# duburcqa/jiminy

Hardware: AMD Instinct MI355X
Metric: env-steps/s (whole node) ANYmal 18-DoF batch 65536; achieved HBM GB/s vs peak (higher is better)
Workload: dtype f64

## Files before the change

### jiminy_amd/csrc/jm_quad.h

```cpp
#pragma once
#include "jm_kernels.h"

namespace jm
{
template<class Tp> struct QLayout
{
    static constexpr int J_PLC = 0, J_RBI = 12, J_AXIS = 22, J_AXP = 25, J_ROTOR = 28, J_QLO = 29, J_QHI = 30, J_MOTOR = 31, J_ENC = 40;
    static constexpr int QJ = 41;
    static constexpr int C_IDX = 12, C_CS = 13, C_FREL = 14;
    static constexpr int QC = Tp::QHAS_FORCE ? 26 : 14;
    static constexpr int CONTACT = Tp::QN * QJ;
    static constexpr int RAW = CONTACT + Tp::QCL * QC;
    static constexpr int QSTRIDE = (RAW % 2 == 0) ? RAW + 1 : RAW;
    static constexpr int TABLE = 4 * QSTRIDE;
    static constexpr int OFFSET = Layout<Tp>::TOTAL;
    static constexpr int TOTAL = OFFSET + TABLE;
};

JM_DEV int sel4(int k, int c0, int c1, int c2, int c3) { return k == 0 ? c0 : (k == 1 ? c1 : (k == 2 ? c2 : c3)); }

template<class Tp> struct QInfo
{
    static constexpr int N = Tp::QN, NT = Tp::QT;
    static constexpr int NQB = 7 + (NT - 1), NVB = 6 + (NT - 1);
// ... 44 lines not shown
    if (ax == 1) return {c * R.m00 - s * R.m02, R.m01, c * R.m02 + s * R.m00, c * R.m10 - s * R.m12, R.m11, c * R.m12 + s * R.m10,
                         c * R.m20 - s * R.m22, R.m21, c * R.m22 + s * R.m20};
    return {c * R.m00 + s * R.m01, c * R.m01 - s * R.m00, R.m02, c * R.m10 + s * R.m11, c * R.m11 - s * R.m10, R.m12,
            c * R.m20 + s * R.m21, c * R.m21 - s * R.m20, R.m22};
}
template<class T> struct LimbTable
{
    const T * base;
    JM_DEV T operator()(int off) const { return base[off]; }
    JM_DEV V3<T> v3(int o) const { return {base[o], base[o + 1], base[o + 2]}; }
    JM_DEV M3<T> m3(int o) const { return {base[o], base[o + 1], base[o + 2], base[o + 3], base[o + 4], base[o + 5], base[o + 6], base[o + 7], base[o + 8]}; }
    JM_DEV SE3<T> se3(int o) const { return {m3(o), v3(o + 9)}; }
    JM_DEV RBI<T> rbi(int o) const { return {base[o], v3(o + 1), S3<T>{base[o + 4], base[o + 5], base[o + 6], base[o + 7], base[o + 8], base[o + 9]}}; }
};
template<class T, class Tp, int s> JM_DEV V3<T> limb_axis_root(const LimbTable<T> & LT, const M3<T> & Rs_)
{
    constexpr int ax = limb_axis_uniform<Tp>(s);
    if constexpr (ax >= 0)
    {
        if constexpr (limb_axis_negative<Tp>(s)) return LT(s * QLayout<Tp>::QJ + QLayout<Tp>::J_AXIS + ax) * mcol(Rs_, ax);
        else return mcol(Rs_, ax);
    }
    else return Rs_ * LT.v3(s * QLayout<Tp>::QJ + QLayout<Tp>::J_AXIS);
}

template<class T, class X> JM_DEV Sp<T> quad_sum6(Sp<T> a)
{
    return {{X::quad_sum(a.l.x), X::quad_sum(a.l.y), X::quad_sum(a.l.z)}, {X::quad_sum(a.a.x), X::quad_sum(a.a.y), X::quad_sum(a.a.z)}};
}
template<class T, class X> JM_DEV AI<T> quad_sum_ai(const AI<T> & Y)
{
    AI<T> r;
    r.A = {X::quad_sum(Y.A.xx), X::quad_sum(Y.A.xy), X::quad_sum(Y.A.xz), X::quad_sum(Y.A.yy), X::quad_sum(Y.A.yz), X::quad_sum(Y.A.zz)};
    r.B = {X::quad_sum(Y.B.m00), X::quad_sum(Y.B.m01), X::quad_sum(Y.B.m02), X::quad_sum(Y.B.m10), X::quad_sum(Y.B.m11), X::quad_sum(Y.B.m12),
           X::quad_sum(Y.B.m20), X::quad_sum(Y.B.m21), X::quad_sum(Y.B.m22)};
    r.D = {X::quad_sum(Y.D.xx), X::quad_sum(Y.D.xy), X::quad_sum(Y.D.xz), X::quad_sum(Y.D.yy), X::quad_sum(Y.D.yz), X::quad_sum(Y.D.zz)};
    return r;
}
template<class T> JM_DEV Sp<T> operator*(T s, Sp<T> a) { return {s * a.l, s * a.a}; }
template<class T> JM_DEV T dot6(Sp<T> a, Sp<T> b) { return dot(a.l, b.l) + dot(a.a, b.a); }
template<class T> JM_DEV Sp<T> mask6(bool on, Sp<T> a)
{
    const T z = T(0);
    return {{on ? a.l.x : z, on ? a.l.y : z, on ? a.l.z : z}, {on ? a.a.x : z, on ? a.a.y : z, on ? a.a.z : z}};
}
template<class T> JM_DEV AI<T> mask_ai(bool on, const AI<T> & Y)
{
    const T z = T(0);
    AI<T> r;
    r.A = {on ? Y.A.xx : z, on ? Y.A.xy : z, on ? Y.A.xz : z, on ? Y.A.yy : z, on ? Y.A.yz : z, on ? Y.A.zz : z};
    r.B = {on ? Y.B.m00 : z, on ? Y.B.m01 : z, on ? Y.B.m02 : z, on ? Y.B.m10 : z, on ? Y.B.m11 : z, on ? Y.B.m12 : z,
           on ? Y.B.m20 : z, on ? Y.B.m21 : z, on ? Y.B.m22 : z};
    r.D = {on ? Y.D.xx : z, on ? Y.D.xy : z, on ? Y.D.xz : z, on ? Y.D.yy : z, on ? Y.D.yz : z, on ? Y.D.zz : z};
    return r;
}
template<class T> JM_DEV RBI<T> rbi_placed(const M3<T> & R, V3<T> p, const RBI<T> & Y)
{
    return {Y.m, R * Y.c + p, rot_sym(R, Y.I)};
}

template<class T, int SL, int SB> struct StageBuf
{
    T * sl;
    T * sb;
    bool wb;
    JM_DEV T getl(int row) const { return sl[row * SL]; }
    JM_DEV void putl(int row, T x) const { sl[row * SL] = x; }
    JM_DEV T getb(int row) const { return sb[row * SB]; }
    JM_DEV void putb(int row, T x) const { if (wb) sb[row * SB] = x; }
};
template<class Tp> struct QRows
{
    static constexpr int N = Tp::QN, NQB = QInfo<Tp>::NQB, NVB = QInfo<Tp>::NVB;
    static constexpr int Q0B = 0, V0B = NQB, ACCVB = V0B + NVB, ACCAB = ACCVB + NVB, KVB = ACCAB + NVB;
    static constexpr int Q0L = 0, V0L = N, ACCVL = 2 * N, ACCAL = 3 * N, KVL = 4 * N;
#ifdef JM_QUAD_LEAN
    static constexpr bool LONG = true;
#else
    static constexpr bool LONG = N > 4;
#endif
    static constexpr bool CMD_LDS = true;
    static constexpr int CMDL = 5 * N, NL = CMD_LDS ? 6 * N : 5 * N;
    static constexpr int CMDB = KVB + NVB, NB = CMD_LDS ? CMDB + Tp::QT : CMDB;
};

template<class Tp> struct QSplitRows
{
    using R = QRows<Tp>;
    static constexpr int N = Tp::QN, NQB = QInfo<Tp>::NQB, NVB = QInfo<Tp>::NVB;
    static constexpr int CURQL = R::NL, CURVL = CURQL + N, DDQL = CURVL + N, STATUSL = DDQL + N, CXL = STATUSL + 1, NCX = 16;
    static constexpr int NL = CXL + NCX;
    static constexpr int CURQB = R::NB, CURVB = CURQB + NQB, DDQB = CURVB + NVB, NB = DDQB + NVB;
    static constexpr int TILE = NL * 64 + NB * 16;
};

template<class T> JM_DEV void add6(T * base, unsigned B, unsigned r, unsigned row0, Sp<T> f)
{
    const unsigned o = row0 * B + r;
    base[o] += f.l.x; base[o + B] += f.l.y; base[o + 2 * B] += f.l.z;
    base[o + 3 * B] += f.a.x; base[o + 4 * B] += f.a.y; base[o + 5 * B] += f.a.z;
}
template<class T> JM_DEV void put6(T * base, unsigned B, unsigned r, unsigned row0, Sp<T> f)
{
    const unsigned o = row0 * B + r;
    base[o] = f.l.x; base[o + B] = f.l.y; base[o + 2 * B] = f.l.z;
    base[o + 3 * B] = f.a.x; base[o + 4 * B] = f.a.y; base[o + 5 * B] = f.a.z;
}

template<class T, int FL, class MP> JM_DEV void motor_law(MP && mp, T cmd, T vjnt, T & um, T & ut)
{
    const T red = mp(0), elim = mp(1), vlim = mp(2), islope = mp(3);
    const T vmot = red * vjnt;
    um = cmd;
    if constexpr ((FL & JM_MOTOR_EFFORT_LIMIT) != 0)
    {
        T emin = -elim, emax = elim;
        if constexpr ((FL & JM_MOTOR_VELOCITY_LIMIT) != 0)
        {
            const T vdelta = elim * islope;
            const bool on = vdelta > T(0);
            const T vthr = fmax_(vlim - vdelta, T(0));
            const T inv = rcp_(on ? vlim - vthr : T(1));
            emin *= on ? clamp_((vlim + vmot) * inv, T(0), T(1)) : T(1);
            emax *= on ? clamp_((vlim - vmot) * inv, T(0), T(1)) : T(1);
        }
        um = clamp_(um, emin, emax);
    }
    ut = red * um;
    if constexpr ((FL & JM_MOTOR_FRICTION) != 0)
    {
        const T fds = mp(8);
        if (vjnt > T(0)) ut += mp(4) * vjnt + mp(6) * tanh_(fds * vjnt);
        else ut += mp(5) * vjnt + mp(7) * tanh_(fds * vjnt);
    }
}

template<class Tp> struct QIdx
{
    int rq[Tp::QN], rv[Tp::QN], rm[Tp::QN];
    bool has[Tp::QN];
    int nc;
    int attach;
};
template<class Tp> JM_DEV QIdx<Tp> quad_indices(int k)
{
    QIdx<Tp> ix;
    static_for<0, Tp::QN>([&](auto sc) {
        constexpr int s = decltype(sc)::value;
        constexpr auto J = [](int kk) { return Tp::limb_joint[kk][s] < 0 ? 1 : Tp::limb_joint[kk][s]; };
        ix.rq[s] = sel4(k, Tp::idx_q[J(0)], Tp::idx_q[J(1)], Tp::idx_q[J(2)], Tp::idx_q[J(3)]);
        ix.rv[s] = sel4(k, Tp::idx_v[J(0)], Tp::idx_v[J(1)], Tp::idx_v[J(2)], Tp::idx_v[J(3)]);
        ix.rm[s] = sel4(k, Tp::limb_motor[0][s] < 0 ? 0 : Tp::limb_motor[0][s], Tp::limb_motor[1][s] < 0 ? 0 : Tp::limb_motor[1][s],
                        Tp::limb_motor[2][s] < 0 ? 0 : Tp::limb_motor[2][s], Tp::limb_motor[3][s] < 0 ? 0 : Tp::limb_motor[3][s]);
        ix.has[s] = sel4(k, s < Tp::limb_len[0], s < Tp::limb_len[1], s < Tp::limb_len[2], s < Tp::limb_len[3]) != 0;
    });
    ix.nc = sel4(k, Tp::limb_ncontact[0], Tp::limb_ncontact[1], Tp::limb_ncontact[2], Tp::limb_ncontact[3]);
    ix.attach = sel4(k, Tp::limb_attach[0], Tp::limb_attach[1], Tp::limb_attach[2], Tp::limb_attach[3]);
    return ix;
}

struct NoModelLane
{
    template<class V> JM_DEV V rbi(int, const V & c) const { return c; }
    template<class V> JM_DEV V plc_p(int, const V & c) const { return c; }
};
template<class T> struct ModelLane
// ... 303 lines not shown
    constexpr int ax = limb_axis_uniform<Tp>(s);
    if constexpr (ax >= 0)
    {
        R = mul_rot_axis(R * plc.R, ax, c, sn);
        if constexpr (limb_axis_negative<Tp>(s)) a = LT(o + Q::J_AXIS + ax) * mcol(R, ax);
        else a = mcol(R, ax);
    }
    else
    {
        a = R * LT.v3(o + Q::J_AXP);
        R = R * (plc.R * rot_rodrigues(LT.v3(o + Q::J_AXIS), c, sn));
    }
}
template<class T, class Tp, int s, class MA = NoModelLane>
JM_DEV void limb_unwind(const LimbTable<T> & LT, T c, T sn, M3<T> & R, V3<T> & p, const MA & ma = MA{}, int k = 0)
{
    using Q = QLayout<Tp>;
    constexpr int o = s * Q::QJ;
    SE3<T> plc = LT.se3(o + Q::J_PLC);
    if constexpr (!std::is_same<MA, NoModelLane>::value)
        plc.p = ma.plc_p(sel4(k, Tp::limb_joint[0][s], Tp::limb_joint[1][s], Tp::limb_joint[2][s], Tp::limb_joint[3][s]), plc.p);
    constexpr int ax = limb_axis_uniform<Tp>(s);
    M3<T> Rq;
    if constexpr (ax >= 0) Rq = mul_rot_axis(R, ax, c, -sn);
    else Rq = R * rot_rodrigues(LT.v3(o + Q::J_AXIS), c, -sn);
    R = mul_bt(Rq, plc.R);
    p = p - R * plc.p;
}

template<class T> JM_DEV Sp<T> applied_wrench_on(const BatchArgs<T> & A, int jq, const M3<T> & R1, const M3<T> & Rj, V3<T> pj,
                                                 unsigned B32, unsigned r32, T te)
{
    Sp<T> f = zero6<T>();
    for (int i = 0; i < A.applied_k; ++i)
    {
        if (A.applied_joint[i] != jq) continue;
        V3<T> F = zero3<T>(), M = zero3<T>();
        if (A.applied)
        {
            const unsigned o = (unsigned)(6 * i) * B32 + r32;
            F = {A.applied[o], A.applied[o + B32], A.applied[o + 2 * B32]};
            M = {A.applied[o + 3 * B32], A.applied[o + 4 * B32], A.applied[o + 5 * B32]};
        }
        if (A.proc_off > 0) add_process_forces(A, i, te, (long long)B32, (long long)r32, F, M);
        const V3<T> p = pj + Rj * V3<T>{A.applied_p[3 * i], A.applied_p[3 * i + 1], A.applied_p[3 * i + 2]};
        const V3<T> fl = tmul(R1, F);
        f.l = f.l + fl;
        f.a = f.a + tmul(R1, M) + cross(p, fl);
    }
    return f;
}
template<class T> JM_DEV Sp<T> applied_root_wrench(const BatchArgs<T> & A, const M3<T> & R1, unsigned B32, unsigned r32, T te)
{
    return applied_wrench_on(A, 1, R1, ident3<T>(), zero3<T>(), B32, r32, te);
}
template<class T> JM_DEV Sp<T> wrench_to_joint(const M3<T> & Rj, V3<T> pj, Sp<T> w)
{
    return {tmul(Rj, w.l), tmul(Rj, w.a - cross(pj, w.l))};
}

template<class T, class Tp> struct QExtra
{
    T tau_l[Tp::QN], tau_b[Tp::QT], uemit_l[Tp::QN], uemit_b[Tp::QT];
    bool motors_on;
    const int32_t * flags;
    const T * lam;
    int nb;
};
struct NoKeep { static constexpr bool ON = false; };
template<class T, class Tp> struct TrunkStore;
template<class T, class Tp> struct QKeep
{
    static constexpr bool ON = true;
    V3<T> ps[Tp::QN], as[Tp::QN];
    Sp<T> Us[Tp::QN];
    T dinv[Tp::QN];
    M3<T> Rt;
    Sp<T> vtip, atip;
    M3<T> R1; V3<T> p1;
    Sp<T> agf1;
    T rootL[6][6], rootdinv[6];
};

template<class T, class Tp, class X, bool EMIT, class SB, int CFM = 0, class KEEP = NoKeep, bool GEN = false, bool DYN = true>
JM_DEV void quad_eval(CPtr<T> P, const LimbTable<T> & LT, const BatchArgs<T> & A, unsigned r, int k, const QIdx<Tp> & ix,
                      const SB & S_, const T * qb, const T * vb_, const T * ql, const T * vl_, const T * cmdb_, const T * cmdl_,
                      bool sensors, T * ddqb, T * ddq, int & status, const QExtra<T, Tp> * ex = nullptr, KEEP * keep = nullptr,
                      TrunkStore<T, Tp> * ts_out = nullptr, T te = T(0))
{
    (void)te;
    using RW = QRows<Tp>;
    auto vlq = [&](int s) -> T { if constexpr (RW::LONG) return S_.getl(RW::KVL + s); else return vl_[s]; };
    auto vbq = [&](int i) -> T { if constexpr (RW::LONG) return S_.getb(RW::KVB + i); else return vb_[i]; };
    auto cmdlq = [&](int s) -> T { if constexpr (RW::CMD_LDS) return S_.getl(RW::CMDL + s); else return cmdl_[s]; };
    auto cmdbq = [&](int t) -> T { if constexpr (RW::CMD_LDS) return S_.getb(RW::CMDB + t); else return cmdb_[t]; };
    constexpr bool emit = EMIT;
    using L = Layout<Tp>;
    using Q = QLayout<Tp>;
    using I = QInfo<Tp>;
    constexpr int N = Tp::QN, NT = Tp::QT;
    constexpr int FL = Tp::motor_flags[0];
    const unsigned B32 = (unsigned)A.B;
    unsigned r32 = r;
    JM_OPAQUE(r32);
    unsigned Bg = B32, rg = r32;
    if constexpr (GEN)
        if (A.lane_map) { rg = (unsigned)A.lane_map[r32]; Bg = (unsigned)A.B_full; }
    const bool lead = (k == 0);
    const bool emit_sens = emit && sensors;
    const bool want_energy = emit && A.energy;
    if constexpr (Tp::QHAS_ENC)
        if (emit_sens && A.encoder)
        {
            static_for<0, N>([&](auto sc) {
                constexpr int s = decltype(sc)::value;
                const int si = sel4(k, Tp::limb_enc[0][s], Tp::limb_enc[1][s], Tp::limb_enc[2][s], Tp::limb_enc[3][s]);
                T pos = ql[s], vel = vlq(s);
                if constexpr (Tp::QENC_SIDE == 0)
                {
                    const T red = LT(s * Q::QJ + Q::J_ENC);
                    pos *= red;
                    vel *= red;
                }
                if (ix.has[s])
                {
                    A.encoder[(unsigned)(2 * si) * B32 + r32] = pos;
                    A.encoder[(unsigned)(2 * si + 1) * B32 + r32] = vel;
                }
            });
            if (lead)
                static_for<1, NT>([&](auto tc) {
                    constexpr int t = decltype(tc)::value;
                    constexpr int si = Tp::trunk_enc[t];
                    T pos = qb[6 + t], vel = vbq(5 + t);
                    if constexpr (Tp::QENC_SIDE == 0) { pos *= P[L::ENC + si]; vel *= P[L::ENC + si]; }
                    A.encoder[(unsigned)(2 * si) * B32 + r32] = pos;
                    A.encoder[(unsigned)(2 * si + 1) * B32 + r32] = vel;
                });
        }
    const M3<T> R1 = quat_to_matrix(qb[3], qb[4], qb[5], qb[6]);
    const V3<T> p1 = {qb[0], qb[1], qb[2]};
    V3<T> p1g = p1;
    if constexpr (GEN)
        if (A.ground_off) { p1g.x += A.ground_off[rg]; p1g.y += A.ground_off[Bg + rg]; }
    const V3<T> g = ld_v3<T>(P, L::OPT), gw = ld_v3<T>(P, L::OPT + 3);
    const Sp<T> v1 = {{vb_[0], vb_[1], vb_[2]}, {vb_[3], vb_[4], vb_[5]}};
    const Sp<T> agf1 = actinv_motion(SE3<T>{R1, p1}, Sp<T>{-g, -gw});
    TrunkStore<T, Tp> TS;
#ifdef JM_HOST_EMU
    std::memset(&TS, 0xFF, sizeof(TS));
#endif
    SE3<T> Xatt;
    Sp<T> vatt;
    using MA = std::conditional_t<GEN, ModelLane<T>, NoModelLane>;
    MA ma;
    if constexpr (GEN) ma = ModelLane<T>{A.model_lane, Bg, rg};
    auto limb_joint_of = [&](auto sc) {
        constexpr int s = decltype(sc)::value;
        return sel4(k, Tp::limb_joint[0][s], Tp::limb_joint[1][s], Tp::limb_joint[2][s], Tp::limb_joint[3][s]);
    };
    (void)limb_joint_of;
    trunk_fk_store<T, Tp, X, MA>(P, k, ix, qb, vb_, TS, Xatt, vatt, status, ma);
#ifdef JM_OUTPUT_KEEP_KIN
    constexpr bool UNWIND = QRows<Tp>::LONG;
#else
    constexpr bool UNWIND = QRows<Tp>::LONG || !DYN;
#endif
    constexpr bool REWIND = UNWIND;
    M3<T> Rs[UNWIND ? 1 : N];
    V3<T> ps[N];
    T cq[UNWIND ? N : 1], sq[UNWIND ? N : 1];
    M3<T> Rtip;
    V3<T> ptip;
    Sp<T> vtip;
    if constexpr (UNWIND) limb_fk_tip<T, Tp, MA>(LT, Xatt, vatt, ql, vl_, cq, sq, Rtip, ptip, vtip, status, ma, k);
    else
    {
        limb_fk<T, Tp, MA>(LT, ix, Xatt, vatt, ql, vl_, Rs, ps, vtip, status, ma, k);
        Rtip = Rs[N - 1]; ptip = ps[N - 1];
    }
    if constexpr (CFM != 0) status &= ~JM_LANE_OUT_OF_BOUNDS;
    Sp<T> fext = zero6<T>();
    {
        const M3<T> Rt = Rtip;
        const V3<T> pt = ptip;
        const Sp<T> vt = vtip;
        Sp<T> fext_loc = zero6<T>(), fsens = zero6<T>();
        T fmax2 = T(0);
        auto one_contact = [&](int c) {
            const int oc = Q::CONTACT + c * Q::QC;
            const SE3<T> fr = LT.se3(oc);
            const V3<T> pc = Rt * fr.p + pt;
            T depth = p1.z + dot(V3<T>{R1.m20, R1.m21, R1.m22}, pc);
            V3<T> nG = {T(0), T(0), T(1)};
            if constexpr (GEN && CFM == 0)
                if (A.ground_h)
                {
                    const V3<T> pW = R1 * pc + p1g;
                    T hG;
                    ground_profile(A, pW.x, pW.y, hG, nG);
                    depth = (pW.z - hG) * nG.z;
                }
            const bool active = c < ix.nc;
            Sp<T> fl = zero6<T>();
            if constexpr (CFM == 0)
            {
                if (active && depth < T(0))
                {
                    const V3<T> vW = R1 * (vt.l + cross(vt.a, pc));
                    V3<T> fW;
                    if constexpr (GEN) fW = contact_law_n<T, Tp>(P, nG, depth, vW, A.friction ? A.friction[rg] : T(-1));
                    else fW = contact_law<T, Tp>(P, depth, vW);
                    const V3<T> fR = tmul(R1, fW);
                    fext.l = fext.l + fR;
                    fext.a = fext.a + cross(pc, fR);
                    fmax2 = fmax_(fmax2, dot(fW, fW));
                    if (emit)
                    {
                        fl.l = tmul(Rt, fR);
                        fl.a = cross(fr.p, fl.l);
                    }
                }
            }
            else if constexpr (CFM == 2)
            {
                (void)depth;
                if (active)
                {
                    const unsigned ci = (unsigned)(int)LT(oc + Q::C_IDX);
                    if (ex->flags[((unsigned)ex->nb + ci) * B32 + r32] & 1)
                    {
                        const unsigned o = ((unsigned)ex->nb + 4u * ci) * B32 + r32;
                        T dep_;
                        const M3<T> Mc = contact_frame<GEN>(A, R1, p1g, pc, dep_);
                        const V3<T> fR = tmul(Mc, V3<T>{ex->lam[o], ex->lam[o + B32], ex->lam[o + 2 * B32]});
                        const V3<T> tR = ex->lam[o + 3 * B32] * V3<T>{Mc.m20, Mc.m21, Mc.m22};
                        fext.l = fext.l + fR;
                        fext.a = fext.a + cross(pc, fR) + tR;
                        if (emit)
                        {
                            fl.l = tmul(Rt, fR);
                            fl.a = cross(fr.p, fl.l) + tmul(Rt, tR);
                        }
                    }
                }
            }
            else { (void)depth; }
            if (emit && active)
            {
                fext_loc = fext_loc + fl;
                const Sp<T> cf = actinv_force(fr, fl);
                if (A.contact_forces) put6(A.contact_forces, B32, r32, 6 * (unsigned)(int)LT(oc + Q::C_IDX), cf);
                if constexpr (Tp::QHAS_CS)
                    if (sensors && A.contact)
                    {
                        const unsigned o = 3 * (unsigned)(int)LT(oc + Q::C_CS) * B32 + r32;
                        A.contact[o] = cf.l.x; A.contact[o + B32] = cf.l.y; A.contact[o + 2 * B32] = cf.l.z;
                    }
                if constexpr (Tp::QHAS_FORCE)
                    if (sensors && A.force) fsens = fsens + act_force(LT.se3(oc + Q::C_FREL), cf);
            }
        };
        if constexpr (Tp::QCL <= 2)
            static_for<0, Tp::QCL>([&](auto cc) { one_contact(decltype(cc)::value); });
        else
        {
#pragma nounroll
            for (int c = 0; c < Tp::QCL; ++c) one_contact(c);
        }
        if constexpr (EMIT && CFM == 0)
            if ((A.mode == MODE_START || A.mode == MODE_RESET) && fmax2 > T(1e10)) status |= JM_LANE_FORCE_OVERFLOW;
        if (emit)
        {
            if (A.f_external)
            {
                if (lead)
                {
                    put6(A.f_external, B32, r32, 0, zero6<T>());
                    static_for<0, NT>([&](auto tc) { put6(A.f_external, B32, r32, 6 * Tp::trunk_joint[decltype(tc)::value], zero6<T>()); });
                    if constexpr (GEN)
                        if (A.applied_k > 0) put6(A.f_external, B32, r32, 6 * Tp::trunk_joint[0], applied_root_wrench(A, R1, Bg, rg, te));
                }
                static_for<0, N>([&](auto sc) {
                    constexpr int s = decltype(sc)::value;
                    const int j = sel4(k, Tp::limb_joint[0][s], Tp::limb_joint[1][s], Tp::limb_joint[2][s], Tp::limb_joint[3][s]);
                    const bool tip = sel4(k, s == Tp::limb_len[0] - 1, s == Tp::limb_len[1] - 1, s == Tp::limb_len[2] - 1, s == Tp::limb_len[3] - 1) != 0;
                    if (ix.has[s]) put6(A.f_external, B32, r32, 6 * (unsigned)j, mask6(tip, fext_loc));
                });
            }
            if constexpr (Tp::QHAS_FORCE)
                if (sensors && A.force)
                {
                    const int si = sel4(k, Tp::limb_force[0], Tp::limb_force[1], Tp::limb_force[2], Tp::limb_force[3]);
                    if (si >= 0) put6(A.force, B32, r32, 6 * (unsigned)si, fsens);
                }
        }
    }
    constexpr bool MOTORS_IN_SWEEP = QRows<Tp>::LONG && !EMIT && DYN;
    T u[N], ut[NT];
    auto limb_motor = [&](auto sc) -> T {
        constexpr int s = decltype(sc)::value;
        constexpr int o = s * Q::QJ + Q::J_MOTOR;
        T um, ue;
        motor_law<T, FL>([&](int i) { return LT(o + i); }, cmdlq(s), vlq(s), um, ue);
        T ueff = ue, ue_out = ue;
        if constexpr (CFM != 0)
        {
            ueff = (ex->motors_on ? ue : T(0)) + ex->tau_l[s];
            ue_out = ue + ex->uemit_l[s];
        }
        if (emit && ix.has[s])
        {
            if (A.u_motor) A.u_motor[(unsigned)ix.rm[s] * B32 + r32] = um;
            if (A.u) A.u[(unsigned)ix.rv[s] * B32 + r32] = ue_out;
            if constexpr (Tp::QHAS_EFF)
                if (sensors && A.effort)
                {
                    const int si = sel4(k, Tp::limb_eff[0][s], Tp::limb_eff[1][s], Tp::limb_eff[2][s], Tp::limb_eff[3][s]);
                    A.effort[(unsigned)si * B32 + r32] = um;
                }
        }
        return ueff;
    };
    auto trunk_motor = [&](auto tc) -> T {
        constexpr int t = decltype(tc)::value;
        constexpr int m = Tp::trunk_motor[t];
        constexpr int o = L::MOTOR + JM_MOTOR_NPARAMS * m;
        T um, ue;
        motor_law<T, FL>([&](int i) { return P[o + i]; }, cmdbq(t), vbq(5 + t), um, ue);
        T ueff = ue, ue_out = ue;
        if constexpr (CFM != 0)
        {
            ueff = (ex->motors_on ? ue : T(0)) + ex->tau_b[t];
            ue_out = ue + ex->uemit_b[t];
        }
        if (emit && lead)
        {
            if (A.u_motor) A.u_motor[(unsigned)m * B32 + r32] = um;
            if (A.u) A.u[(unsigned)Tp::idx_v[Tp::trunk_joint[t]] * B32 + r32] = ue_out;
            if constexpr (Tp::QHAS_EFF)
                if (sensors && A.effort) A.effort[(unsigned)Tp::trunk_eff[t] * B32 + r32] = um;
        }
        return ueff;
    };
    if constexpr (!MOTORS_IN_SWEEP)
    {
        static_for<0, N>([&](auto sc) { u[decltype(sc)::value] = limb_motor(sc); });
        ut[0] = T(0);
        static_for<1, NT>([&](auto tc) { ut[decltype(tc)::value] = trunk_motor(tc); });
    }
    if (emit && A.u && lead)
    {
#pragma unroll
        for (int i = 0; i < 6; ++i) A.u[(unsigned)(Tp::idx_v[1] + i) * B32 + r32] = T(0);
    }
    JM_REFRESH();
    constexpr bool KEEP_SC = !QRows<Tp>::LONG;
    V3<T> as[N];
    Sp<T> Ss[KEEP_SC ? N : 1], cs[KEEP_SC ? N : 1];
    Sp<T> Us[N];
    T dinv[N];
    AI<T> Ia;
    Sp<T> pa = zero6<T>();
    T kin = T(0), rot = T(0), msum = T(0);
    V3<T> mc = zero3<T>();
    {
        Sp<T> vcur = vtip;
        M3<T> Rcur = Rtip;
        V3<T> pcur = ptip;
        static_rfor<0, N>([&](auto sc) {
            constexpr int s = decltype(sc)::value;
            constexpr int o = s * Q::QJ;
            if constexpr (!UNWIND) { Rcur = Rs[s]; pcur = ps[s]; }
            else if constexpr (!REWIND) ps[s] = pcur;
            if constexpr (!DYN) return;
            const RBI<T> Y = rbi_placed(Rcur, pcur, ma.rbi(GEN ? limb_joint_of(sc) : 0, LT.rbi(o + Q::J_RBI)));
            const V3<T> a = limb_axis_root<T, Tp, s>(LT, Rcur);
            const Sp<T> S = {cross(pcur, a), a};
            Sp<T> f = cross_mf(vcur, rbi_mul(Y, vcur));
            if constexpr (s == N - 1) { f = f - fext; Ia = ai_from_rbi(Y); }
            else { f = f + pa; Ia = ai_from_rbi(Y) + Ia; }
            if constexpr (GEN)
                if (A.applied_k > 0)
                {
                    const Sp<T> w = applied_wrench_on(A, limb_joint_of(sc), R1, Rcur, pcur, Bg, rg, te);
                    f = f - w;
                    if constexpr (EMIT)
                        if (A.f_external && ix.has[s]) add6(A.f_external, B32, r32, 6u * (unsigned)limb_joint_of(sc), wrench_to_joint(Rcur, pcur, w));
                }
            if (want_energy)
            {
                kin += rbi_vtiv(Y, vcur);
                mc = mc + Y.m * Y.c;
                msum += Y.m;
                rot += LT(o + Q::J_ROTOR) * vlq(s) * vlq(s);
            }
            const Sp<T> vj = vlq(s) * S;
            vcur = vcur - vj;
            const Sp<T> c = cross_mm(vcur, vj);
            if constexpr (MOTORS_IN_SWEEP) u[s] = limb_motor(sc);
            const T uj = u[s] - dot6(S, f);
            const Sp<T> U = ai_mul(Ia, S);
            const T D = dot6(S, U) + LT(o + Q::J_ROTOR);
            const T di = rcp_(D);
            ai_rank1_sub(Ia, U, di);
            const Sp<T> Ya = ai_mul(Ia, c);
            const T ud = uj * di;
            pa = {f.l + Ya.l + ud * U.l, f.a + Ya.a + ud * U.a};
            Us[s] = U; dinv[s] = di; u[s] = uj;
            if constexpr (KEEP_SC) { Ss[s] = S; cs[s] = c; }
            else if constexpr (!REWIND) as[s] = a;
            if constexpr (KEEP::ON) { keep->ps[s] = pcur; keep->as[s] = a; keep->Us[s] = U; keep->dinv[s] = di; }
            if constexpr (UNWIND && s > 0) limb_unwind<T, Tp, s, MA>(LT, cq[s], sq[s], Rcur, pcur, ma, k);
        });
    }
    AI<T> accA[NT];
    Sp<T> accF[NT];
#ifdef JM_HOST_EMU
    std::memset(accA, 0xFF, sizeof(accA)); std::memset(accF, 0xFF, sizeof(accF));
#endif
    if constexpr (DYN)
    static_for<0, NT>([&](auto tc) {
        constexpr int t = decltype(tc)::value;
        if constexpr (I::limb_at(t))
        {
            if constexpr (I::uniform_attach) { accA[t] = quad_sum_ai<T, X>(Ia); accF[t] = quad_sum6<T, X>(pa); }
            else
            {
                const bool mine = ix.attach == t;
                accA[t] = quad_sum_ai<T, X>(mask_ai(mine, Ia));
                accF[t] = quad_sum6<T, X>(mask6(mine, pa));
            }
        }
// ... 762 lines not shown
                static_for<0, NQB>([&](auto ic) { S.putb(R::Q0B + decltype(ic)::value, qb[decltype(ic)::value]); });
                static_for<0, NVB>([&](auto ic) {
                    constexpr int i = decltype(ic)::value;
                    S.putb(R::V0B + i, vb[i]); S.putb(R::KVB + i, vb[i]); S.putb(R::ACCVB + i, T(0)); S.putb(R::ACCAB + i, T(0));
                });
                static_for<0, N>([&](auto sc) {
                    constexpr int s = decltype(sc)::value;
                    S.putl(R::Q0L + s, ql[s]); S.putl(R::V0L + s, vl[s]); S.putl(R::KVL + s, vl[s]);
                    S.putl(R::ACCVL + s, T(0)); S.putl(R::ACCAL + s, T(0));
                });
                if (last)
                {
                    if (lead)
                    {
                        static_for<0, NQB>([&](auto ic) { A.q[(unsigned)I::qrow(decltype(ic)::value) * B32 + rr] = qb[decltype(ic)::value]; });
                        static_for<0, NVB>([&](auto ic) { A.v[(unsigned)I::vrow(decltype(ic)::value) * B32 + rr] = vb[decltype(ic)::value]; });
                    }
                    static_for<0, N>([&](auto sc) {
                        constexpr int s = decltype(sc)::value;
                        if (ix.has[s])
                        {
                            A.q[(unsigned)ix.rq[s] * B32 + rr] = ql[s];
                            A.v[(unsigned)ix.rv[s] * B32 + rr] = vl[s];
                        }
                    });
                }
            }
        }
    };
    unsigned rr = r32;
    if constexpr (QCON)
    {
        const int start_passes = INIT == 1 ? 4 : (INIT == 0 ? (A.mode == MODE_REFRESH ? -1 : 0) :
                                 ((A.mode == MODE_START || A.mode == MODE_RESET) ? 4 : (A.mode == MODE_REFRESH ? -1 : 0)));
        if constexpr (PH != 0)
        {
            const int e = split_e;
            const int st = (e < pre) ? -1 : (rk4 ? ((e - pre) & 3) : 3);
            const bool last = e == n_evals - 1;
            if constexpr (PH == 1)
            {
                advance(st, last, rr);
                static_for<0, NQB>([&](auto ic) { S.putb(SR::CURQB + decltype(ic)::value, qb[decltype(ic)::value]); });
                static_for<0, NVB>([&](auto ic) { S.putb(SR::CURVB + decltype(ic)::value, vb[decltype(ic)::value]); });
                static_for<0, N>([&](auto sc) {
                    S.putl(SR::CURQL + decltype(sc)::value, ql[decltype(sc)::value]);
                    S.putl(SR::CURVL + decltype(sc)::value, vl[decltype(sc)::value]);
                });
            }
            quad_eval_con<T, Tp, X, StageBuf<T, SL, SB>, CAPC, GEN, PH, INIT>(P, LT, A, *C, *V, rr, k, ix, S, qb, vb, ql, vl, cmdb, cmdl, last,
                                    !stepping || A.update_sensors != 0, ddqb, ddq, status,
                                    INIT == 1 ? 4 : (INIT == 0 ? 0 : ((A.mode == MODE_START || A.mode == MODE_RESET) ? 4 : 0)));
            if (PH == 1 || !last)
            {
                S.putl(SR::STATUSL, (T)status);
                if constexpr (PH == 2)
                {
                    static_for<0, NVB>([&](auto ic) { S.putb(SR::DDQB + decltype(ic)::value, ddqb[decltype(ic)::value]); });
                    static_for<0, N>([&](auto sc) { S.putl(SR::DDQL + decltype(sc)::value, ddq[decltype(sc)::value]); });
                }
                return;
            }
        }
        else
        {
#pragma nounroll
        for (int e = 0; e < n_evals; ++e)
        {
            const int st = (e < pre) ? -1 : (rk4 ? ((e - pre) & 3) : 3);
            const bool last = e == n_evals - 1;
            JM_REFRESH();
            rr = r32;
            JM_OPAQUE(rr);
            advance(st, last, rr);
            if (stepping) stage_time(st);
            quad_eval_con<T, Tp, X, StageBuf<T, SL, SB>, CAPC, GEN, 0, INIT>(P, LT, A, *C, *V, rr, k, ix, S, qb, vb, ql, vl, cmdb, cmdl, last && A.mode != MODE_DYNAMICS,
                                    (!stepping && A.mode != MODE_REFRESH) || A.update_sensors != 0, ddqb, ddq, status,
                                    start_passes, te);
        }
        }
    }
    else
    {
    if (stepping)
    {
#pragma nounroll
        for (int e = 0; e < n_evals; ++e)
        {
            const int st = (e < pre) ? -1 : (rk4 ? ((e - pre) & 3) : 3);
            JM_REFRESH();
            rr = r32;
            JM_OPAQUE(rr);
            CPtr<T> Pl = P;
            if constexpr (R::LONG && !GEN) JM_OPAQUE_S(Pl);
            advance(st, e == n_evals - 1, rr);
            stage_time(st);
            quad_eval<T, Tp, X, false, StageBuf<T, SL, SB>, 0, NoKeep, GEN>(Pl, LT, A, rr, k, ix, S, qb, vb, ql, vl, cmdb, cmdl, false, ddqb, ddq, status,
                                                                             nullptr, nullptr, nullptr, te);
        }
    }
    else
    {
        JM_REFRESH();
        rr = r32;
        JM_OPAQUE(rr);
        advance(-1, true, rr);
        quad_eval<T, Tp, X, false, StageBuf<T, SL, SB>, 0, NoKeep, GEN>(P, LT, A, rr, k, ix, S, qb, vb, ql, vl, cmdb, cmdl, false, ddqb, ddq, status,
                                                                         nullptr, nullptr, nullptr, te);
    }
    if (A.mode != MODE_DYNAMICS)
    {
        JM_REFRESH();
        rr = r32;
        JM_OPAQUE(rr);
        static_for<0, NQB>([&](auto ic) { qb[decltype(ic)::value] = S.getb(R::Q0B + decltype(ic)::value); });
        static_for<0, NVB>([&](auto ic) { vb[decltype(ic)::value] = S.getb(R::V0B + decltype(ic)::value); });
        static_for<0, N>([&](auto sc) { ql[decltype(sc)::value] = S.getl(R::Q0L + decltype(sc)::value); vl[decltype(sc)::value] = S.getl(R::V0L + decltype(sc)::value); });
        quad_eval<T, Tp, X, true, StageBuf<T, SL, SB>, 0, NoKeep, GEN, false>(P, LT, A, rr, k, ix, S, qb, vb, ql, vl, cmdb, cmdl,
                                  (!stepping && A.mode != MODE_REFRESH) || A.update_sensors != 0, ddqb, ddq, status,
                                  nullptr, nullptr, nullptr, te);
    }
    }
    {
        T * adst = (A.mode == MODE_DYNAMICS) ? A.a_out : A.a;
        if (lead) static_for<0, NVB>([&](auto ic) { adst[(unsigned)I::vrow(decltype(ic)::value) * B32 + rr] = ddqb[decltype(ic)::value]; });
        static_for<0, N>([&](auto sc) { if (ix.has[decltype(sc)::value]) adst[(unsigned)ix.rv[decltype(sc)::value] * B32 + rr] = ddq[decltype(sc)::value]; });
        if (A.mode != MODE_DYNAMICS)
        {
            const int stq = X::quad_or(status);
            if (A.status && lead) A.status[rr] = (A.mode == MODE_REFRESH) ? (A.status[rr] | stq) : stq;
            if constexpr (GEN && PH == 0)
                if (stepping && lead && A.proc_off > 0) proc_block(A).lane_time()[rr] = tl;
            if constexpr (QCON)
            if (A.joint_forces || A.centroidal)
            {
                JM_REFRESH();
                static_for<0, NQB>([&](auto ic) { qb[decltype(ic)::value] = S.getb(R::Q0B + decltype(ic)::value); });
                static_for<0, NVB>([&](auto ic) { vb[decltype(ic)::value] = S.getb(R::V0B + decltype(ic)::value); });
                static_for<0, N>([&](auto sc) { ql[decltype(sc)::value] = S.getl(R::Q0L + decltype(sc)::value); vl[decltype(sc)::value] = S.getl(R::V0L + decltype(sc)::value); });
                QExtra<T, Tp> ex;
                ex.flags = C->flags;
                ex.nb = qcon_first_contact_row<Tp>();
                ex.lam = C->data + (size_t)qcon_first_lambda_row<Tp>() * B32;
                quad_extra_terms<T, Tp, X, 2, GEN>(P, LT, A, rr, k, ix, qb, vb, ql, vl, ddqb, ddq, &ex, te);
            }
        }
    }
}

#ifndef JM_HOST_EMU
struct DppQuad
{
    template<int CTRL> static __device__ __forceinline__ int mov(int v) { return __builtin_amdgcn_update_dpp(0, v, CTRL, 0xf, 0xf, true); }
    template<int CTRL> static __device__ __forceinline__ double perm(double x)
    {
        const int lo = mov<CTRL>(__double2loint(x)), hi = mov<CTRL>(__double2hiint(x));
        return __hiloint2double(hi, lo);
    }
    template<int CTRL> static __device__ __forceinline__ float perm(float x) { return __int_as_float(mov<CTRL>(__float_as_int(x))); }
    template<int CTRL> static __device__ __forceinline__ int perm(int x) { return mov<CTRL>(x); }
    template<class T> static __device__ __forceinline__ T quad_sum(T x)
    {
        x = x + perm<0xB1>(x);
        x = x + perm<0x4E>(x);
        return x;
    }
    template<int LANE, class T> static __device__ __forceinline__ T bcast(T x) { return perm<LANE * 0x55>(x); }
    static __device__ __forceinline__ int quad_or(int x)
    {
        x |= mov<0xB1>(x);
        x |= mov<0x4E>(x);
        return x;
    }
    template<int CTRL, class T> static __device__ __forceinline__ T perm_(T x) { return perm<CTRL>(x); }
    static __device__ __forceinline__ bool wave_any(bool p) { return __builtin_amdgcn_ballot_w64(p) != 0ull; }
    static __device__ __forceinline__ double max_abs(double a, double b)
    {
        double r;
        asm("v_max_f64 %0, %1, |%2|" : "=v"(r) : "v"(a), "v"(b));
        return r;
    }
    static __device__ __forceinline__ double max_(double a, double b)
    {
        double r;
        asm("v_max_f64 %0, %1, %2" : "=v"(r) : "v"(a), "v"(b));
        return r;
    }
    static __device__ __forceinline__ float max_abs(float a, float b) { return fmaxf(a, fabsf(b)); }
    static __device__ __forceinline__ float max_(float a, float b) { return fmaxf(a, b); }
#ifdef JM_SYNC_FENCE
    static __device__ __forceinline__ void sync() { __builtin_amdgcn_fence(__ATOMIC_ACQ_REL, "wavefront"); }
#else
    static __device__ __forceinline__ void sync() {}
#endif
    static __device__ __forceinline__ void fence() { __builtin_amdgcn_fence(__ATOMIC_SEQ_CST, "workgroup"); }
    static __device__ __forceinline__ void table_ready() { __syncthreads(); }
};

template<class T, class Tp> constexpr int quad_block_waves()
{
#ifdef JM_QUAD_BLOCK_WAVES
    return JM_QUAD_BLOCK_WAVES;
#endif
    constexpr long per_wave = (long)sizeof(T) * (QRows<Tp>::NL * 64 + QRows<Tp>::NB * 16);
    constexpr long table = (long)sizeof(T) * QLayout<Tp>::TABLE;
    int best = 1, best_resident = 0;
    for (int w = 1; w <= 4; w *= 2)
    {
        long blocks = (160L * 1024) / (table + w * per_wave);
// ... 52 lines not shown
```

Measured before the change: 455.1 million.

## Emit quad sensor, contact and motor outputs during final dynamics eval

For short-limb, single-trunk quadruped configurations, the last RK stage (or the single eval) now writes encoder, contact-force, f_external, force-sensor, u and u_motor outputs directly. It also stashes the summed tip wrench in LDS. The later emit pass (QE_OUT) then reuses that wrench and skips the contact and motor recomputation. Accelerations are written before the output pass. The aim is to remove redundant contact and actuator work in the refresh/emit evaluation. The cost is extra branches, register pressure and code size inside the hot eval loop.

```diff
diff --git a/jiminy_amd/csrc/jm_quad.h b/jiminy_amd/csrc/jm_quad.h
--- a/jiminy_amd/csrc/jm_quad.h
+++ b/jiminy_amd/csrc/jm_quad.h
@@ -150,6 +150,7 @@
     static constexpr bool CMD_LDS = true;
     static constexpr int CMDL = 5 * N, NL = CMD_LDS ? 6 * N : 5 * N;
     static constexpr int CMDB = KVB + NVB, NB = CMD_LDS ? CMDB + Tp::QT : CMDB;
+    static constexpr int FEXTL = ACCVL;
 };
 
 template<class Tp> struct QSplitRows
@@ -619,13 +620,25 @@
     T rootL[6][6], rootdinv[6];
 };
 
-template<class T, class Tp, class X, bool EMIT, class SB, int CFM = 0, class KEEP = NoKeep, bool GEN = false, bool DYN = true>
+enum { QE_OFF = 0, QE_LOOP = 1, QE_SINGLE = 2, QE_OUT = 3 };
+template<class Tp, bool GEN, bool QCON, int CFM = 0, class KEEP = NoKeep> constexpr bool quad_early_outputs()
+{
+#ifdef JM_QUAD_NO_EARLY_OUTPUTS
+    return false;
+#endif
+    return !GEN && !QCON && CFM == 0 && !KEEP::ON && !QRows<Tp>::LONG && Tp::QT == 1 && 2 * Tp::QN >= 6;
+}
+
+template<class T, class Tp, class X, bool EMIT, class SB, int CFM = 0, class KEEP = NoKeep, bool GEN = false, bool DYN = true, int EARLY = QE_OFF>
 JM_DEV void quad_eval(CPtr<T> P, const LimbTable<T> & LT, const BatchArgs<T> & A, unsigned r, int k, const QIdx<Tp> & ix,
                       const SB & S_, const T * qb, const T * vb_, const T * ql, const T * vl_, const T * cmdb_, const T * cmdl_,
                       bool sensors, T * ddqb, T * ddq, int & status, const QExtra<T, Tp> * ex = nullptr, KEEP * keep = nullptr,
-                      TrunkStore<T, Tp> * ts_out = nullptr, T te = T(0))
+                      TrunkStore<T, Tp> * ts_out = nullptr, T te = T(0), bool early = false)
 {
     (void)te;
+    (void)early;
+    constexpr bool EARLY_DYN = EARLY == QE_LOOP || EARLY == QE_SINGLE, EARLY_OUT = EARLY == QE_OUT;
+    static_assert(EARLY == QE_OFF || (quad_early_outputs<Tp, GEN, false, CFM, KEEP>() && (EARLY_DYN ? (DYN && !EMIT) : (!DYN && EMIT))), "early outputs: wrong kernel form");
     using RW = QRows<Tp>;
     auto vlq = [&](int s) -> T { if constexpr (RW::LONG) return S_.getl(RW::KVL + s); else return vl_[s]; };
     auto vbq = [&](int i) -> T { if constexpr (RW::LONG) return S_.getb(RW::KVB + i); else return vb_[i]; };
@@ -646,7 +659,30 @@
     const bool lead = (k == 0);
     const bool emit_sens = emit && sensors;
     const bool want_energy = emit && A.energy;
-    if constexpr (Tp::QHAS_ENC)
+    if constexpr (Tp::QHAS_ENC && EARLY_DYN)
+        if (early && sensors && A.encoder)
+        {
+            int ke = k;
+            JM_OPAQUE(ke);
+            const QIdx<Tp> ixe = quad_indices<Tp>(ke);
+            static_for<0, Tp::QN>([&](auto sc) {
+                constexpr int s = decltype(sc)::value;
+                const int si = sel4(ke, Tp::limb_enc[0][s], Tp::limb_enc[1][s], Tp::limb_enc[2][s], Tp::limb_enc[3][s]);
+                T pos = ql[s], vel = vl_[s];
+                if constexpr (Tp::QENC_SIDE == 0)
+                {
+                    const T red = LT(s * QLayout<Tp>::QJ + QLayout<Tp>::J_ENC);
+                    pos *= red;
+                    vel *= red;
+                }
+                if (ixe.has[s])
+                {
+                    A.encoder[(unsigned)(2 * si) * B32 + r32] = pos;
+                    A.encoder[(unsigned)(2 * si + 1) * B32 + r32] = vel;
+                }
+            });
+        }
+    if constexpr (Tp::QHAS_ENC && !EARLY_OUT)
         if (emit_sens && A.encoder)
         {
             static_for<0, N>([&](auto sc) {
@@ -718,6 +754,9 @@
     }
     if constexpr (CFM != 0) status &= ~JM_LANE_OUT_OF_BOUNDS;
     Sp<T> fext = zero6<T>();
+    if constexpr (EARLY_OUT)
+        fext = {{S_.getl(RW::FEXTL), S_.getl(RW::FEXTL + 1), S_.getl(RW::FEXTL + 2)}, {S_.getl(RW::FEXTL + 3), S_.getl(RW::FEXTL + 4), S_.getl(RW::FEXTL + 5)}};
+    if constexpr (!EARLY_OUT)
     {
         const M3<T> Rt = Rtip;
         const V3<T> pt = ptip;
@@ -757,6 +796,12 @@
                         fl.l = tmul(Rt, fR);
                         fl.a = cross(fr.p, fl.l);
                     }
+                    if constexpr (EARLY_DYN)
+                        if (early)
+                        {
+                            fl.l = tmul(Rt, fR);
+                            fl.a = cross(fr.p, fl.l);
+                        }
                 }
             }
             else if constexpr (CFM == 2)
@@ -797,6 +842,21 @@
                 if constexpr (Tp::QHAS_FORCE)
                     if (sensors && A.force) fsens = fsens + act_force(LT.se3(oc + Q::C_FREL), cf);
             }
+            if constexpr (EARLY_DYN)
+                if (early && active)
+                {
+                    fext_loc = fext_loc + fl;
+                    const Sp<T> cf = actinv_force(fr, fl);
+                    if (A.contact_forces) put6(A.contact_forces, B32, r32, 6 * (unsigned)(int)LT(oc + Q::C_IDX), cf);
+                    if constexpr (Tp::QHAS_CS)
+                        if (sensors && A.contact)
+                        {
+                            const unsigned o = 3 * (unsigned)(int)LT(oc + Q::C_CS) * B32 + r32;
+                            A.contact[o] = cf.l.x; A.contact[o + B32] = cf.l.y; A.contact[o + 2 * B32] = cf.l.z;
+                        }
+                    if constexpr (Tp::QHAS_FORCE)
+                        if (sensors && A.force) fsens = fsens + act_force(LT.se3(oc + Q::C_FREL), cf);
+                }
         };
         if constexpr (Tp::QCL <= 2)
             static_for<0, Tp::QCL>([&](auto cc) { one_contact(decltype(cc)::value); });
@@ -807,6 +867,37 @@
         }
         if constexpr (EMIT && CFM == 0)
             if ((A.mode == MODE_START || A.mode == MODE_RESET) && fmax2 > T(1e10)) status |= JM_LANE_FORCE_OVERFLOW;
+        if constexpr (EARLY_DYN)
+            if (early)
+            {
+                if constexpr (EARLY == QE_SINGLE)
+                    if ((A.mode == MODE_START || A.mode == MODE_RESET) && fmax2 > T(1e10)) status |= JM_LANE_FORCE_OVERFLOW;
+                S_.putl(RW::FEXTL, fext.l.x); S_.putl(RW::FEXTL + 1, fext.l.y); S_.putl(RW::FEXTL + 2, fext.l.z);
+                S_.putl(RW::FEXTL + 3, fext.a.x); S_.putl(RW::FEXTL + 4, fext.a.y); S_.putl(RW::FEXTL + 5, fext.a.z);
+                int ke = k;
+                JM_OPAQUE(ke);
+                const QIdx<Tp> ixe = quad_indices<Tp>(ke);
+                if (A.f_external)
+                {
+                    if (ke == 0)
+                    {
+                        put6(A.f_external, B32, r32, 0, zero6<T>());
+                        static_for<0, NT>([&](auto tc) { put6(A.f_external, B32, r32, 6 * Tp::trunk_joint[decltype(tc)::value], zero6<T>()); });
+                    }
+                    static_for<0, N>([&](auto sc) {
+                        constexpr int s = decltype(sc)::value;
+                        const int j = sel4(ke, Tp::limb_joint[0][s], Tp::limb_joint[1][s], Tp::limb_joint[2][s], Tp::limb_joint[3][s]);
+                        const bool tip = sel4(ke, s == Tp::limb_len[0] - 1, s == Tp::limb_len[1] - 1, s == Tp::limb_len[2] - 1, s == Tp::limb_len[3] - 1) != 0;
+                        if (ixe.has[s]) put6(A.f_external, B32, r32, 6 * (unsigned)j, mask6(tip, fext_loc));
+                    });
+                }
+                if constexpr (Tp::QHAS_FORCE)
+                    if (sensors && A.force)
+                    {
+                        const int si = sel4(ke, Tp::limb_force[0], Tp::limb_force[1], Tp::limb_force[2], Tp::limb_force[3]);
+                        if (si >= 0) put6(A.force, B32, r32, 6 * (unsigned)si, fsens);
+                    }
+            }
         if (emit)
         {
             if (A.f_external)
@@ -846,6 +937,24 @@
             ueff = (ex->motors_on ? ue : T(0)) + ex->tau_l[s];
             ue_out = ue + ex->uemit_l[s];
         }
+        if constexpr (EARLY_DYN)
+            if (early)
+            {
+                int ke = k;
+                JM_OPAQUE(ke);
+                const QIdx<Tp> ixe = quad_indices<Tp>(ke);
+                if (ixe.has[s])
+                {
+                    if (A.u_motor) A.u_motor[(unsigned)ixe.rm[s] * B32 + r32] = um;
+                    if (A.u) A.u[(unsigned)ixe.rv[s] * B32 + r32] = ue_out;
+                    if constexpr (Tp::QHAS_EFF)
+                        if (sensors && A.effort)
+                        {
+                            const int si = sel4(ke, Tp::limb_eff[0][s], Tp::limb_eff[1][s], Tp::limb_eff[2][s], Tp::limb_eff[3][s]);
+                            A.effort[(unsigned)si * B32 + r32] = um;
+                        }
+                }
+            }
         if (emit && ix.has[s])
         {
             if (A.u_motor) A.u_motor[(unsigned)ix.rm[s] * B32 + r32] = um;
@@ -880,12 +989,24 @@
         }
         return ueff;
     };
-    if constexpr (!MOTORS_IN_SWEEP)
+    if constexpr (!MOTORS_IN_SWEEP && !EARLY_OUT)
     {
         static_for<0, N>([&](auto sc) { u[decltype(sc)::value] = limb_motor(sc); });
         ut[0] = T(0);
         static_for<1, NT>([&](auto tc) { ut[decltype(tc)::value] = trunk_motor(tc); });
     }
+    if constexpr (EARLY_DYN)
+        if (early && A.u)
+        {
+            int ke = k;
+            JM_OPAQUE(ke);
+            if (ke == 0)
+            {
+#pragma unroll
+                for (int i = 0; i < 6; ++i) A.u[(unsigned)(Tp::idx_v[1] + i) * B32 + r32] = T(0);
+            }
+        }
+    if constexpr (!EARLY_OUT)
     if (emit && A.u && lead)
     {
 #pragma unroll
@@ -1814,6 +1935,7 @@
     }
     else
     {
+    constexpr bool EARLY = quad_early_outputs<Tp, GEN, QCON>();
     if (stepping)
     {
 #pragma nounroll
@@ -1827,6 +1949,10 @@
             if constexpr (R::LONG && !GEN) JM_OPAQUE_S(Pl);
             advance(st, e == n_evals - 1, rr);
             stage_time(st);
+            if constexpr (EARLY)
+                quad_eval<T, Tp, X, false, StageBuf<T, SL, SB>, 0, NoKeep, GEN, true, QE_LOOP>(Pl, LT, A, rr, k, ix, S, qb, vb, ql, vl, cmdb, cmdl, A.update_sensors != 0,
+                                                                                 ddqb, ddq, status, nullptr, nullptr, nullptr, te, e == n_evals - 1);
+            else
             quad_eval<T, Tp, X, false, StageBuf<T, SL, SB>, 0, NoKeep, GEN>(Pl, LT, A, rr, k, ix, S, qb, vb, ql, vl, cmdb, cmdl, false, ddqb, ddq, status,
                                                                              nullptr, nullptr, nullptr, te);
         }
@@ -1837,6 +1963,11 @@
         rr = r32;
         JM_OPAQUE(rr);
         advance(-1, true, rr);
+        if constexpr (EARLY)
+            quad_eval<T, Tp, X, false, StageBuf<T, SL, SB>, 0, NoKeep, GEN, true, QE_SINGLE>(P, LT, A, rr, k, ix, S, qb, vb, ql, vl, cmdb, cmdl,
+                                      A.mode != MODE_REFRESH || A.update_sensors != 0, ddqb, ddq, status, nullptr, nullptr, nullptr, te,
+                                      A.mode != MODE_DYNAMICS);
+        else
         quad_eval<T, Tp, X, false, StageBuf<T, SL, SB>, 0, NoKeep, GEN>(P, LT, A, rr, k, ix, S, qb, vb, ql, vl, cmdb, cmdl, false, ddqb, ddq, status,
                                                                          nullptr, nullptr, nullptr, te);
     }
@@ -1845,9 +1976,19 @@
         JM_REFRESH();
         rr = r32;
         JM_OPAQUE(rr);
+        if constexpr (EARLY)
+        {
+            if (lead) static_for<0, NVB>([&](auto ic) { A.a[(unsigned)I::vrow(decltype(ic)::value) * B32 + rr] = ddqb[decltype(ic)::value]; });
+            static_for<0, N>([&](auto sc) { if (ix.has[decltype(sc)::value]) A.a[(unsigned)ix.rv[decltype(sc)::value] * B32 + rr] = ddq[decltype(sc)::value]; });
+        }
         static_for<0, NQB>([&](auto ic) { qb[decltype(ic)::value] = S.getb(R::Q0B + decltype(ic)::value); });
         static_for<0, NVB>([&](auto ic) { vb[decltype(ic)::value] = S.getb(R::V0B + decltype(ic)::value); });
         static_for<0, N>([&](auto sc) { ql[decltype(sc)::value] = S.getl(R::Q0L + decltype(sc)::value); vl[decltype(sc)::value] = S.getl(R::V0L + decltype(sc)::value); });
+        if constexpr (EARLY)
+            quad_eval<T, Tp, X, true, StageBuf<T, SL, SB>, 0, NoKeep, GEN, false, QE_OUT>(P, LT, A, rr, k, ix, S, qb, vb, ql, vl, cmdb, cmdl,
+                                      (!stepping && A.mode != MODE_REFRESH) || A.update_sensors != 0, ddqb, ddq, status,
+                                      nullptr, nullptr, nullptr, te);
+        else
         quad_eval<T, Tp, X, true, StageBuf<T, SL, SB>, 0, NoKeep, GEN, false>(P, LT, A, rr, k, ix, S, qb, vb, ql, vl, cmdb, cmdl,
                                   (!stepping && A.mode != MODE_REFRESH) || A.update_sensors != 0, ddqb, ddq, status,
                                   nullptr, nullptr, nullptr, te);
@@ -1855,8 +1996,19 @@
     }
     {
         T * adst = (A.mode == MODE_DYNAMICS) ? A.a_out : A.a;
+        if constexpr (quad_early_outputs<Tp, GEN, QCON>())
+        {
+            if (A.mode == MODE_DYNAMICS)
+            {
+                if (lead) static_for<0, NVB>([&](auto ic) { adst[(unsigned)I::vrow(decltype(ic)::value) * B32 + rr] = ddqb[decltype(ic)::value]; });
+                static_for<0, N>([&](auto sc) { if (ix.has[decltype(sc)::value]) adst[(unsigned)ix.rv[decltype(sc)::value] * B32 + rr] = ddq[decltype(sc)::value]; });
+            }
+        }
+        else
+        {
         if (lead) static_for<0, NVB>([&](auto ic) { adst[(unsigned)I::vrow(decltype(ic)::value) * B32 + rr] = ddqb[decltype(ic)::value]; });
         static_for<0, N>([&](auto sc) { if (ix.has[decltype(sc)::value]) adst[(unsigned)ix.rv[decltype(sc)::value] * B32 + rr] = ddq[decltype(sc)::value]; });
+        }
         if (A.mode != MODE_DYNAMICS)
         {
             const int stq = X::quad_or(status);
```

Result: no change. 462.1 million, median of 3 (+1.5%).
